# zeahmed/NeuralASR

Hardware: AMD Instinct MI355X
Metric: audio-frames/sec (fwd+bwd+CTC+Adam) at batch 16 per GPU (higher is better)
Workload: dtype f32

## Files before the change

### neuralasr_amd/csrc/lstm_persist.hip

```cpp
#include "kernels.h"
#include "lstm_device.h"

#include <cstdlib>

#ifndef NASR_PSTAMP
#define NASR_PSTAMP 0
#endif

namespace nasr {

namespace {

struct Stamps {
  unsigned long long last;
  unsigned acc[12];
  bool on;
  __device__ __forceinline__ void start(bool enable) {
    on = enable;
    for (int i = 0; i < 12; ++i) acc[i] = 0;
    last = NASR_PSTAMP ? __builtin_amdgcn_s_memtime() : 0ull;
  }
  __device__ __forceinline__ void mark(int i) {
#if NASR_PSTAMP
    if (on) {
      const unsigned long long t = __builtin_amdgcn_s_memtime();
      acc[i] += (unsigned)(t - last);
      last = t;
    }
#endif
  }
  __device__ __forceinline__ void flush(PersistCtl* ctl, unsigned slot, bool first) {
#if NASR_PSTAMP
    if (on && (threadIdx.x & 63) == 0) {
      for (int i = 0; i < 12; ++i) ctl->stamps[slot & 255][i] = acc[i];
      if (first)
        for (int i = 0; i < 12; ++i) ctl->pad[i] = acc[i];
    }
#endif
  }
};

__device__ __forceinline__ void raise_error(PersistCtl* ctl, unsigned* sticky, float* fault, unsigned code) {
  atomicOr(&ctl->error, code);
  if (fault) *fault = 1.f;
  if (sticky) __hip_atomic_store(sticky, code, __ATOMIC_RELAXED, __HIP_MEMORY_SCOPE_SYSTEM);
}

__device__ __forceinline__ bool join_group(PersistCtl* ctl, unsigned* sticky, float* fault, unsigned* info, unsigned& xcc,
                                           unsigned& member) {
  if (threadIdx.x == 0) {
    const unsigned x = __builtin_amdgcn_s_getreg((3 << 11) | 20) & 15u;
    info[0] = x;
    info[1] = x < 8 ? atomicAdd(&ctl->xcc_count[x], 1u) : 0xffffu;
    info[2] = 0;
    info[3] = 0;
    info[4] = 0;
    info[5] = 0;
  }
  __syncthreads();
  xcc = info[0];
  member = info[1];
  if (xcc >= 8 || member >= 32) {
    if (threadIdx.x == 0) raise_error(ctl, sticky, fault, 2u);
    return false;
  }
  return true;
}

}

struct RepackOffs { long long o[PERSIST_MAX_MATS]; };
__global__ __launch_bounds__(256) void repack_persist_kernel(const float* __restrict__ P, RepackOffs off,
                                                             float* __restrict__ Upf0, float* __restrict__ Upb0,
                                                             long long imf, long long imb, int Hp,
                                                             const float* __restrict__ cs0) {
  const float* __restrict__ U = P + off.o[blockIdx.y];
  float* __restrict__ Upf = Upf0 + (size_t)blockIdx.y * imf;
  float* __restrict__ Upb = Upb0 + (size_t)blockIdx.y * imb;
  const int NU = Hp / 32, KW = 8 * NU, N4 = 4 * Hp;
  const int NOG = (KW + 63) / 64, KB = NOG * 4 * NU;
  const int64_t nf = (int64_t)32 * 4 * KW * 64, nb = (int64_t)32 * 4 * KB * 64;
  const int64_t nfe = cs0 ? nf / 4 : nf;
  (void)nb; (void)Upb; (void)KB;
  for (int64_t e0 = blockIdx.x * (int64_t)blockDim.x + threadIdx.x; e0 < nfe; e0 += (int64_t)gridDim.x * blockDim.x) {
    {
      const int lane = e0 & 63;
      int64_t x = e0 >> 6;
      const int KWe = cs0 ? KW / 4 : KW;
      const int idx = (int)(x % KWe) * (cs0 ? 4 : 1); x /= KWe;
      const int w = (int)(x & 3), m = (int)(x >> 2);
      const int bp = lane >> 2, g = lane & 3;
      if (!cs0) {
        Upf[e0] = bp < NU ? U[(size_t)(w * KW + idx) * N4 + 4 * (NU * m + bp) + g] : 0.f;
      } else {
        const int col = 4 * (NU * m + bp) + g;
        const float sc = bp < NU ? cs0[(size_t)blockIdx.y * N4 + col] : 1.f;
        typedef _Float16 h4 __attribute__((ext_vector_type(4)));
        h4 p1, p2;
#pragma unroll
        for (int r = 0; r < 4; ++r) {
          const float v = bp < NU ? U[(size_t)(w * KW + idx + r) * N4 + col] * sc : 0.f;
          const _Float16 h1 = (_Float16)v;
          p1[r] = h1;
          p2[r] = (_Float16)(v - (float)h1);
        }
        h4* dst = reinterpret_cast<h4*>(Upf) + ((((size_t)m * 4 + w) * (KW / 4) + idx / 4) * 2) * 64 + lane;
        dst[0] = p1;
        dst[64] = p2;
      }
    }
  }
}

__global__ __launch_bounds__(256) void repack_persist_bwd_kernel(const float* __restrict__ P, RepackOffs off,
                                                                 float* __restrict__ Upb0, long long imb, int Hp) {
  __shared__ float tile[64][65];
  const float* __restrict__ U = P + off.o[blockIdx.y];
  float* __restrict__ Upb = Upb0 + (size_t)blockIdx.y * imb;
  const int NU = Hp / 32, KW = 8 * NU, N4 = 4 * Hp, NC = 4 * NU;
  const int NOG = (KW + 63) / 64, KB = NOG * NC;
  const int og = blockIdx.x % NOG, w = (blockIdx.x / NOG) & 3, m = blockIdx.x / (NOG * 4);
  const int cx = threadIdx.x & 63, ry = threadIdx.x >> 6;
  for (int r = ry; r < 64; r += 4) {
    const int kl = og * 64 + r;
    tile[r][cx] = (kl < KW && cx < NC) ? U[(size_t)(w * KW + kl) * N4 + NC * m + cx] : 0.f;
  }
  __syncthreads();
  float* dst = Upb + (((size_t)m * 4 + w) * KB + (size_t)og * NC) * 64;
  for (int c = ry; c < NC; c += 4) dst[(size_t)c * 64 + cx] = tile[cx][c];
}

size_t persist_image_floats(int Hp, bool bwd) {
  const int NU = Hp / 32, KW = 8 * NU, NOG = (KW + 63) / 64;
  return (size_t)32 * 4 * 64 * (bwd ? NOG * 4 * NU : KW);
}

void launch_repack_persist(const float* P, const int64_t* offs, int n, float* Upf, float* Upb, int Hp, const float* col_scale,
                           hipStream_t st) {
  const long long imf = (long long)persist_image_floats(Hp, false), imb = (long long)persist_image_floats(Hp, true);
  for (int k0 = 0; k0 < n; k0 += PERSIST_MAX_MATS) {
    const int m = n - k0 < PERSIST_MAX_MATS ? n - k0 : PERSIST_MAX_MATS;
    RepackOffs off{};
    for (int k = 0; k < m; ++k) off.o[k] = offs[k0 + k];
    hipLaunchKernelGGL(repack_persist_kernel, dim3(512, m), dim3(256), 0, st, P, off, Upf + (size_t)k0 * imf,
                       Upb + (size_t)k0 * imb, imf, imb, Hp, col_scale ? col_scale + (size_t)k0 * 4 * Hp : nullptr);
    const int NU = Hp / 32, NOG = (8 * NU + 63) / 64;
    hipLaunchKernelGGL(repack_persist_bwd_kernel, dim3(32 * 4 * NOG, m), dim3(256), 0, st, P, off, Upb + (size_t)k0 * imb, imb, Hp);
  }
}

struct PersistGeom {
  int T, Bp, Hp, D;
  int ub;
  int rounds;
  int inject;
  float* fault;
};

constexpr int PERSIST_LDS_BYTES = 96 * 1024;
constexpr int PERSIST_LDS_LEAN = 24 * 1024;

constexpr int LDS_RED = 0, LDS_ADG = 2 * 4 * 4 * 64, LDS_SIDE = LDS_ADG + 2 * 256, LDS_XGB = LDS_SIDE + 2 * 64 * 8,
              LDS_PFB = LDS_XGB + 2 * 64 * 4, LDS_INFO = LDS_PFB + 2 * 64 * 8;


template <int NU, bool F16>
__global__ __launch_bounds__(320, 1) void lstm_persist_fwd_kernel(
    const float* __restrict__ Upf,
    float* gates, float* cbuf, float* out, const int* __restrict__ seq_len,
    float* hx,
    PersistCtl* ctl, unsigned* sticky, PersistGeom gm, float fb, const float* __restrict__ cinv) {
  extern __shared__ __attribute__((aligned(16))) float lds[];
  constexpr int KW = 8 * NU;
  constexpr int NCH = 2 * NU;
  constexpr int NJ = (NCH + 15) / 16;
  constexpr bool EP = F16;
  float* red = lds + LDS_RED;
  float* side = lds + LDS_SIDE;
  float* xgb = lds + LDS_XGB;
  unsigned* info = reinterpret_cast<unsigned*>(lds + LDS_INFO);
  const int tid = threadIdx.x, w = tid >> 6, lane = tid & 63;
  unsigned xcc, member;
  if (!join_group(ctl, sticky, gm.fault, info, xcc, member)) return;
  const int T = gm.T, Bp = gm.Bp, Hp = gm.Hp, D = gm.D;
  const int NGD = 8 / D, d = (int)xcc / NGD, grp = (int)xcc % NGD;
  const int N4 = 4 * Hp, DH = D * Hp, DN = D * N4;
  if (w < 4) __builtin_amdgcn_s_setprio(3);

  typedef _Float16 h4 __attribute__((ext_vector_type(4)));
  float wreg[F16 ? 1 : KW];
  h4 w1[F16 ? KW / 4 : 1], w2[F16 ? KW / 4 : 1];
  float oscale = 1.f;
  if (w < 4) {
    if constexpr (F16) {
      const h4* wp = reinterpret_cast<const h4*>(Upf) + ((((size_t)d * 32 + member) * 4 + w) * (KW / 4) * 2) * 64 + lane;
#pragma unroll
      for (int i = 0; i < KW / 4; ++i) { w1[i] = wp[(size_t)(2 * i) * 64]; w2[i] = wp[(size_t)(2 * i + 1) * 64]; }
      const int bp = lane >> 2, g = lane & 3;
      oscale = (bp < NU ? cinv[(size_t)d * 4 * gm.Hp + 4 * (NU * (int)member + bp) + g] : 1.f) * (1.f / 16384.f);
    } else {
      const float* wp = Upf + ((((size_t)d * 32 + member) * 4 + w) * KW) * 64 + lane;
#pragma unroll
      for (int i = 0; i < KW; ++i) wreg[i] = wp[(size_t)i * 64];
    }
  }
  float* ghx = hx + (size_t)xcc * 2 * Hp * 4;
  gu32* gflag = (gu32*)(ctl->flags + xcc * 128);

  const int q = lane >> 4, u = lane & 15;
  const bool lane_ok = u < NU;
  const int j = NU * (int)member + u;
  const int jcl = j < Hp ? j : Hp - 1;
  const int hidx = (j >> 2) * 16 + q * 4 + (j & 3);
  bool aborted = false;
  Stamps stp;
  stp.start(w == 0);
  auto epoch_of = [&](int rd, int s) -> unsigned { return (unsigned)(rd * ((T + 1 - (s & 1)) >> 1) + (s >> 1) + 1) & 1u; };

  for (int rd = 0; rd < gm.rounds; ++rd) {
    const int b0 = (rd * NGD + grp) * gm.ub;
    if (b0 >= Bp) continue;
    const int b = b0 + q;
    const bool rowok = lane_ok && q < gm.ub && b < Bp;
    const int bcl = b < Bp ? b : Bp - 1;
    const int len = rowok ? seq_len[b] : 0;
    const unsigned tagbase = (unsigned)(rd * T);
    float c = 0.f;
    const unsigned xoff = (unsigned)bcl * (unsigned)DN + (unsigned)(d * N4 + 4 * jcl), xstep = (unsigned)Bp * (unsigned)DN;
    auto frame_of = [&](int s) { return (rowok && s < len) ? (d ? len - 1 - s : s) : 0; };
    auto load_xg = [&](int s) { return *reinterpret_cast<const f32x4*>(gates + (xoff + (unsigned)frame_of(s) * xstep)); };
    f32x4 xg_pf = (f32x4){0.f, 0.f, 0.f, 0.f};
    if (w == 4) xg_pf = load_xg(0);
    auto store_side = [&](int s) {
      if (rowok) {
        if (s < len) {
          const float* sp = side + ((s & 1) * 64 + lane) * 8;
          const f32x4 act = *reinterpret_cast<const f32x4*>(sp);
          const float2 ch = *reinterpret_cast<const float2*>(sp + 4);
          const unsigned r = (unsigned)((d ? (len - 1 - s) : s) * Bp + b);
          *reinterpret_cast<f32x4*>(gates + (r * (unsigned)DN + (unsigned)(d * N4 + 4 * j))) = act;
          const unsigned oc = r * (unsigned)DH + (unsigned)(d * Hp + j);
          cbuf[oc] = ch.x;
          out[oc] = ch.y;
        } else {
          out[(unsigned)(s * Bp + b) * (unsigned)DH + (unsigned)(d * Hp + j)] = 0.f;
        }
      }
    };
    for (int s = 0; s < T; ++s) {
      const int par = s & 1;
      stp.mark(0);
      bool ok = true;
      if (w < 4) {
        f32x4 acc[4];
#pragma unroll
        for (int i = 0; i < 4; ++i) acc[i] = (f32x4){0.f, 0.f, 0.f, 0.f};
        f32x4 P[NJ];
#pragma unroll
        for (int i = 0; i < NJ; ++i) P[i] = (f32x4){0.f, 0.f, 0.f, 0.f};
        if constexpr (EP) {
          if (s == 0 && rd > 0) ok = poll_ge(gflag + w * 8 + (lane & 7), lane < 8, tagbase);
          if (s == gm.inject && member == 0) ok = false;
          stp.mark(1);
          if (s > 0 && ok) {
            if (w > 0) {
              const unsigned want = tagbase + (unsigned)s;
              for (unsigned n = 0; n < (1u << 26) && (int)(*(lds_vu32*)(info + 5) - want) < 0; ++n) __builtin_amdgcn_s_sleep(1);
            }
            const float* src = ghx + (size_t)((s - 1) & 1) * Hp * 4 + ((size_t)w * KW * 4 + (size_t)lane * 4);
            const unsigned eexp = epoch_of(rd, s - 1) << 30;
            const bool has0 = NCH >= 16 || lane < 4 * NCH, has1 = NJ == 2 && lane < 4 * (NCH - 16);
            bool need = true;
            ok = false;
            for (unsigned n = 0; n < SPIN_BUDGET; ++n) {
              if (need) {
                if (has0) asm volatile("global_load_dwordx4 %0, %1, off sc1" : "=&v"(P[0]) : "v"(src) : "memory");
                if constexpr (NJ == 2)
                  if (has1) asm volatile("global_load_dwordx4 %0, %1, off offset:1024 sc1" : "=&v"(P[NJ - 1]) : "v"(src) : "memory");
              }
              if constexpr (NJ == 2) asm volatile("s_waitcnt vmcnt(0)" : "+v"(P[0]), "+v"(P[NJ - 1]) : : "memory");
              else asm volatile("s_waitcnt vmcnt(0)" : "+v"(P[0]) : : "memory");
              unsigned bad = 0;
              if (has0)
                bad |= (__float_as_uint(P[0][0]) ^ eexp) | (__float_as_uint(P[0][1]) ^ eexp) | (__float_as_uint(P[0][2]) ^ eexp) |
                       (__float_as_uint(P[0][3]) ^ eexp);
              if constexpr (NJ == 2)
                if (has1)
                  bad |= (__float_as_uint(P[NJ - 1][0]) ^ eexp) | (__float_as_uint(P[NJ - 1][1]) ^ eexp) |
                         (__float_as_uint(P[NJ - 1][2]) ^ eexp) | (__float_as_uint(P[NJ - 1][3]) ^ eexp);
              need = (bad & 0x40000000u) != 0;
              if (!__any(need)) { ok = true; break; }
#if NASR_PSTAMP
              if (stp.on) stp.acc[11] += 1;
#endif
            }
          }
        } else {
        ok = poll_ge(gflag + w * 8 + (lane & 7), lane < 8, tagbase + (unsigned)s) && !(s == gm.inject && member == 0);
        stp.mark(1);
        if (s > 0 && ok) {
          const float* src = ghx + (size_t)((s - 1) & 1) * Hp * 4 + ((size_t)w * KW * 4 + (size_t)lane * 4);
          if constexpr (NCH == 32) {
            asm volatile(
                "global_load_dwordx4 %0, %2, off sc1\n\tglobal_load_dwordx4 %1, %2, off offset:1024 sc1\n\ts_waitcnt vmcnt(0)"
                : "=&v"(P[0]), "=&v"(P[1])
                : "v"(src)
                : "memory");
          } else if constexpr (NJ == 2) {
            asm volatile("global_load_dwordx4 %0, %1, off sc1" : "=&v"(P[0]) : "v"(src) : "memory");
            if (lane < 4 * (NCH - 16)) asm volatile("global_load_dwordx4 %0, %1, off offset:1024 sc1" : "=&v"(P[1]) : "v"(src) : "memory");
            asm volatile("s_waitcnt vmcnt(0)" : "+v"(P[0]), "+v"(P[1]) : : "memory");
          } else {
            if (lane < 4 * NCH)
              asm volatile("global_load_dwordx4 %0, %1, off sc1\n\ts_waitcnt vmcnt(0)" : "=&v"(P[0]) : "v"(src) : "memory");
          }
        }
        }
        if (w == 0 && lane == 0) *(lds_vu32*)(info + 4) = tagbase + (unsigned)s + 1u;
        stp.mark(2);
        if (s > 0 && ok) {
          if constexpr (F16) {
            h4 a1[NJ], a2[NJ];
#pragma unroll
            for (int i = 0; i < NJ; ++i) {
              typedef unsigned u2 __attribute__((ext_vector_type(2)));
              const unsigned d0 = __float_as_uint(P[i][0]), d1 = __float_as_uint(P[i][1]);
              const unsigned d2 = __float_as_uint(P[i][2]), d3 = __float_as_uint(P[i][3]);
              const u2 lo = {__builtin_amdgcn_perm(d1, d0, 0x05040100u), __builtin_amdgcn_perm(d3, d2, 0x05040100u)};
              const u2 hi = {__builtin_amdgcn_perm(d1, d0, 0x07060302u), __builtin_amdgcn_perm(d3, d2, 0x07060302u)};
              a1[i] = __builtin_bit_cast(h4, lo);
              a2[i] = __builtin_bit_cast(h4, (u2){hi[0] & 0xBFFFBFFFu, hi[1] & 0xBFFFBFFFu});
            }
            static_for<0, NCH>([&](auto bbc) {
              constexpr int bb = decltype(bbc)::value;
              acc[0] = __builtin_amdgcn_mfma_f32_4x4x4f16(a2[bb / 16], w1[bb], acc[0], 4, bb % 16, 0);
              acc[1] = __builtin_amdgcn_mfma_f32_4x4x4f16(a1[bb / 16], w2[bb], acc[1], 4, bb % 16, 0);
              acc[2] = __builtin_amdgcn_mfma_f32_4x4x4f16(a1[bb / 16], w1[bb], acc[2], 4, bb % 16, 0);
            });
          } else {
            static_for<0, NCH>([&](auto bbc) {
              constexpr int bb = decltype(bbc)::value;
              static_for<0, 4>([&](auto rc) {
                constexpr int r = decltype(rc)::value;
                acc[r] = __builtin_amdgcn_mfma_f32_4x4x1f32(P[bb / 16][r], wreg[bb * 4 + r], acc[r], 4, bb % 16, 0);
              });
            });
          }
        }
        if constexpr (EP) acc[0] *= 8.f;
        f32x4 sum = (acc[0] + acc[1]) + (acc[2] + acc[3]);
        if constexpr (F16) sum *= oscale;
        float* rw = red + ((par * 4 + w) * 4) * 64 + lane;
        rw[0] = sum[0]; rw[64] = sum[1]; rw[128] = sum[2]; rw[192] = sum[3];
        if (!ok) info[2 + par] = 1;
      } else {
        *reinterpret_cast<f32x4*>(xgb + (par * 64 + lane) * 4) = xg_pf;
        const unsigned want = tagbase + (unsigned)s + 1u;
        for (unsigned n = 0; n < (1u << 26) && (int)(*(lds_vu32*)(info + 4) - want) < 0; ++n)
          __builtin_amdgcn_s_sleep(1);
        if (s + 1 < T) xg_pf = load_xg(s + 1);
        if (s > 0) store_side(s - 1);
      }
      stp.mark(3);
#if NASR_PSTAMP
      if (lane == 0) info[8 + w] = (unsigned)__builtin_amdgcn_s_memtime();
#endif
      __syncthreads();
      stp.mark(4);
#if NASR_PSTAMP
      if (stp.on) for (int i = 1; i < 5; ++i) stp.acc[6 + i] += info[8 + i] - info[8];
#endif
      const unsigned abort_word = info[2 + par];
      if (w == 0) {
        const bool valid = rowok && s < len;
        float h = 0.f;
        if (lane_ok) {
          const float* rr = red + (par * 4 * 4 + q) * 64 + 4 * u;
          const f32x4 g0 = *reinterpret_cast<const f32x4*>(rr);
          const f32x4 g1 = *reinterpret_cast<const f32x4*>(rr + 256);
          const f32x4 g2 = *reinterpret_cast<const f32x4*>(rr + 512);
          const f32x4 g3 = *reinterpret_cast<const f32x4*>(rr + 768);
          const f32x4 xg = *reinterpret_cast<const f32x4*>(xgb + (par * 64 + lane) * 4);
          const f32x4 pre = xg + ((g0 + g1) + (g2 + g3));
          f32x4 act;
          act.x = sigmoidf_(pre.x);
          act.y = tanhf_(pre.y);
          act.z = sigmoidf_(pre.z + fb);
          act.w = sigmoidf_(pre.w);
          if (valid) {
            c = c * act.z + act.x * act.y;
            h = tanhf_(c) * act.w;
          }
          if constexpr (F16) {
            const float v = h * 16384.f;
            const _Float16 h1 = (_Float16)v;
            const _Float16 h2 = (_Float16)((v - (float)h1) * 0.125f);
            const unsigned pk = (unsigned)__builtin_bit_cast(unsigned short, h1) |
                                ((unsigned)__builtin_bit_cast(unsigned short, h2) << 16) | (epoch_of(rd, s) << 30);
            ghx[(size_t)par * Hp * 4 + hidx] = __uint_as_float(pk);
          } else {
            ghx[(size_t)par * Hp * 4 + hidx] = h;
          }
          float* sp = side + (par * 64 + lane) * 8;
          *reinterpret_cast<f32x4*>(sp) = act;
          *reinterpret_cast<float2*>(sp + 4) = make_float2(c, h);
        }
        stp.mark(5);
        if constexpr (EP) {
          if (lane == 0) *(lds_vu32*)(info + 5) = tagbase + (unsigned)s + 1u;
        } else {
          asm volatile("s_waitcnt vmcnt(0)" ::: "memory");
        }
        stp.mark(6);
        if (lane == 0) *(ctl->flags + xcc * 128 + member) = tagbase + (unsigned)s + 1u;
      }
      if (abort_word) { aborted = true; break; }
    }
    if (aborted) break;
    __syncthreads();
    if (w == 4) store_side(T - 1);
  }
  stp.flush(ctl, xcc * 32 + member, xcc == 0 && member == 0);
  if (aborted && tid == 0) raise_error(ctl, sticky, gm.fault, 1u);
}

template <int NU>
__global__ __launch_bounds__(320, 1) void lstm_persist_bwd_kernel(
    const float* __restrict__ Upb, const float* __restrict__ gates, float* dgbuf, const float* __restrict__ cbuf,
    const float* __restrict__ dout, const int* __restrict__ seq_len,
    float* px,
    PersistCtl* ctl, unsigned* sticky, PersistGeom gm,
    float* __restrict__ rowpart, float* __restrict__ colpart) {
  extern __shared__ __attribute__((aligned(16))) float lds[];
  constexpr int KW = 8 * NU;
  constexpr int NOG = (KW + 63) / 64;
  constexpr int NC = 4 * NU;
  constexpr int NV = (NC + 15) / 16;
  float* adg = lds + LDS_ADG;
  float* pfb = lds + LDS_PFB;
  unsigned* info = reinterpret_cast<unsigned*>(lds + LDS_INFO);
  const int tid = threadIdx.x, w = tid >> 6, lane = tid & 63;
  unsigned xcc, member;
  if (!join_group(ctl, sticky, gm.fault, info, xcc, member)) return;
  const int T = gm.T, Bp = gm.Bp, Hp = gm.Hp, D = gm.D;
  const int NGD = 8 / D, d = (int)xcc / NGD, grp = (int)xcc % NGD;
  const int N4 = 4 * Hp, DH = D * Hp, DN = D * N4;
  if (w < 4) __builtin_amdgcn_s_setprio(3);

  float wreg[NOG * NC];
  if (w < 4) {
    const float* wp = Upb + ((((size_t)d * 32 + member) * 4 + w) * (NOG * NC)) * 64 + lane;
#pragma unroll
    for (int i = 0; i < NOG * NC; ++i) wreg[i] = wp[(size_t)i * 64];
  }
  float* gpx = px + (size_t)xcc * 2 * 32 * 32 * 64;
  gu32* gflag = (gu32*)(ctl->flags + xcc * 128);

  const int q = lane & 3, u = lane >> 2;
  const bool lane_ok = u < NU;
  const int j = NU * (int)member + u;
  const int jcl = j < Hp ? j : Hp - 1;
  bool aborted = false;
  Stamps stp;
  stp.start(w == 0);
  f32x4 cmax = (f32x4){0.f, 0.f, 0.f, 0.f};
  auto epoch_of = [&](int rd, int k) -> unsigned { return (unsigned)(rd * ((T + 1 - (k & 1)) >> 1) + (k >> 1) + 1) & 1u; };

  for (int rd = 0; rd < gm.rounds; ++rd) {
    const int b0 = (rd * NGD + grp) * gm.ub;
    if (b0 >= Bp) continue;
    const int b = b0 + q;
    const bool rowok = lane_ok && q < gm.ub && b < Bp;
    const int bcl = b < Bp ? b : Bp - 1;
    const int len = rowok ? seq_len[b] : 0;
    const unsigned tagbase = (unsigned)(rd * T);
    float dc = 0.f;
    f32x4 pa = (f32x4){0.f, 0.f, 0.f, 0.f};
    f32x4 pb = (f32x4){0.f, 0.f, 0.f, 0.f};
    auto prefetch = [&](int s) {
      const bool v = rowok && s < len;
      const int tb = v ? (d ? (len - 1 - s) : s) : 0;
      const unsigned r = (unsigned)(tb * Bp + bcl);
      const unsigned rp = (v && s > 0) ? (d ? r + (unsigned)Bp : r - (unsigned)Bp) : r;
      const unsigned cj = (unsigned)(d * Hp + jcl);
      pa = *reinterpret_cast<const f32x4*>(gates + (r * (unsigned)DN + (unsigned)(d * N4 + 4 * jcl)));
      pb.x = cbuf[r * (unsigned)DH + cj];
      pb.y = cbuf[rp * (unsigned)DH + cj];
      pb.z = dout[r * (unsigned)DH + cj];
    };
    auto hand_over = [&](int k) {
      float* dst = pfb + ((k & 1) * 64 + lane) * 8;
      *reinterpret_cast<f32x4*>(dst) = pa;
      *reinterpret_cast<f32x4*>(dst + 4) = pb;
    };
    auto store_dg = [&](int k) {
      float m = 0.f;
      unsigned row = 0;
      if (rowok) {
        const int s = T - 1 - k;
        const float* ad = adg + (k & 1) * 256 + 16 * u + q;
        const f32x4 dg = (f32x4){ad[0], ad[4], ad[8], ad[12]};
        row = (unsigned)(((s < len) ? (d ? (len - 1 - s) : s) : s) * Bp + b);
        *reinterpret_cast<f32x4*>(dgbuf + (row * (unsigned)DN + (unsigned)(d * N4 + 4 * j))) = dg;
        const f32x4 ab = (f32x4){fabsf(dg.x), fabsf(dg.y), fabsf(dg.z), fabsf(dg.w)};
        cmax = (f32x4){fmaxf(cmax.x, ab.x), fmaxf(cmax.y, ab.y), fmaxf(cmax.z, ab.z), fmaxf(cmax.w, ab.w)};
        m = fmaxf(fmaxf(ab.x, ab.y), fmaxf(ab.z, ab.w));
      }
      if (rowpart) {
        m = fmaxf(m, __builtin_bit_cast(float, __builtin_amdgcn_update_dpp(0, __builtin_bit_cast(int, m), 0x124, 0xf, 0xf, false)));
        m = fmaxf(m, __builtin_bit_cast(float, __builtin_amdgcn_update_dpp(0, __builtin_bit_cast(int, m), 0x128, 0xf, 0xf, false)));
        m = fmaxf(m, __shfl_xor(m, 16));
        m = fmaxf(m, __shfl_xor(m, 32));
        if (lane < 4 && rowok) rowpart[(size_t)(d * 32 + (int)member) * ((size_t)T * Bp) + row] = m;
      }
    };
    if (w == 4) {
      prefetch(T - 1);
      hand_over(0);
      if (T > 1) prefetch(T - 2);
    }
    __syncthreads();
    for (int k = 0; k < T; ++k) {
      const int s = T - 1 - k, par = k & 1;
      stp.mark(0);
      if (w == 0) {
        bool ok = false;
        if (k == 0 && rd > 0) {
          const unsigned want = tagbase + (unsigned)k;
          for (unsigned n = 0; n < SPIN_BUDGET && !ok; ++n) {
            const unsigned v0 = __hip_atomic_load(gflag + lane, __ATOMIC_RELAXED, __HIP_MEMORY_SCOPE_AGENT);
            const unsigned v1 = __hip_atomic_load(gflag + 64 + lane, __ATOMIC_RELAXED, __HIP_MEMORY_SCOPE_AGENT);
            ok = __all((int)(v0 - want) >= 0 && (int)(v1 - want) >= 0);
          }
        } else {
          ok = true;
        }
        if (k == gm.inject && member == 0) ok = false;
        stp.mark(1);
        const bool valid = rowok && s < len;
        const float* pf = pfb + (par * 64 + lane) * 8;
        const f32x4 a = *reinterpret_cast<const f32x4*>(pf);
        const f32x4 o = *reinterpret_cast<const f32x4*>(pf + 4);
        float dhs = o.z;
        if (k > 0 && ok) {
          const float* src = gpx + ((size_t)(((k - 1) & 1) * 32 + member) * 32) * 64 + lane;
          float pv[32];
#pragma unroll
          for (int p = 0; p < 32; ++p) pv[p] = 0.f;
#define NASR_LD8(g8)                                                                                               \
  asm volatile(                                                                                                    \
      "global_load_dword %0, %8, off sc1\n\tglobal_load_dword %1, %8, off offset:256 sc1\n\t"                       \
      "global_load_dword %2, %8, off offset:512 sc1\n\tglobal_load_dword %3, %8, off offset:768 sc1\n\t"            \
      "global_load_dword %4, %8, off offset:1024 sc1\n\tglobal_load_dword %5, %8, off offset:1280 sc1\n\t"          \
      "global_load_dword %6, %8, off offset:1536 sc1\n\tglobal_load_dword %7, %8, off offset:1792 sc1"              \
      : "=&v"(pv[g8 + 0]), "=&v"(pv[g8 + 1]), "=&v"(pv[g8 + 2]), "=&v"(pv[g8 + 3]), "=&v"(pv[g8 + 4]),             \
        "=&v"(pv[g8 + 5]), "=&v"(pv[g8 + 6]), "=&v"(pv[g8 + 7])                                                    \
      : "v"(src + (size_t)(g8) * 64)                                                                               \
      : "memory")
          const unsigned eexp = epoch_of(rd, k - 1);
          bool need = lane_ok;
          bool got = false;
          for (unsigned n = 0; n < SPIN_BUDGET; ++n) {
            if (need) { NASR_LD8(0); NASR_LD8(8); NASR_LD8(16); NASR_LD8(24); }
            asm volatile("s_waitcnt vmcnt(0)"
                         : "+v"(pv[0]), "+v"(pv[1]), "+v"(pv[2]), "+v"(pv[3]), "+v"(pv[4]), "+v"(pv[5]), "+v"(pv[6]),
                           "+v"(pv[7]), "+v"(pv[8]), "+v"(pv[9]), "+v"(pv[10]), "+v"(pv[11]), "+v"(pv[12]), "+v"(pv[13]),
                           "+v"(pv[14]), "+v"(pv[15])
                         :
                         : "memory");
            asm volatile(""
                         : "+v"(pv[16]), "+v"(pv[17]), "+v"(pv[18]), "+v"(pv[19]), "+v"(pv[20]), "+v"(pv[21]), "+v"(pv[22]),
                           "+v"(pv[23]), "+v"(pv[24]), "+v"(pv[25]), "+v"(pv[26]), "+v"(pv[27]), "+v"(pv[28]), "+v"(pv[29]),
                           "+v"(pv[30]), "+v"(pv[31])
                         :
                         : "memory");
            unsigned bad;
            if (eexp) {
              unsigned a_ = 1u;
#pragma unroll
              for (int p = 0; p < 32; ++p) a_ &= __float_as_uint(pv[p]);
              bad = ~a_;
            } else {
              unsigned o_ = 0u;
#pragma unroll
              for (int p = 0; p < 32; ++p) o_ |= __float_as_uint(pv[p]);
              bad = o_;
            }
            need = lane_ok && (bad & 1u) != 0;
            if (!__any(need)) { got = true; break; }
#if NASR_PSTAMP
            if (stp.on) stp.acc[11] += 1;
#endif
          }
#undef NASR_LD8
          if (!got) ok = false;
          if (lane_ok) {
            float s0 = 0.f, s1 = 0.f, s2 = 0.f, s3 = 0.f;
#pragma unroll
            for (int p = 0; p < 32; p += 4) { s0 += pv[p]; s1 += pv[p + 1]; s2 += pv[p + 2]; s3 += pv[p + 3]; }
            dhs += (s0 + s1) + (s2 + s3);
          }
        }
        stp.mark(2);
        f32x4 dg = (f32x4){0.f, 0.f, 0.f, 0.f};
        float dcn = 0.f;
        if (valid) {
          const float tc = tanhf_(o.x);
          const float dct = dc + dhs * a.w * (1.f - tc * tc);
          dg.x = dct * a.y * a.x * (1.f - a.x);
          dg.y = dct * a.x * (1.f - a.y * a.y);
          dg.z = dct * (s > 0 ? o.y : 0.f) * a.z * (1.f - a.z);
          dg.w = dhs * tc * a.w * (1.f - a.w);
          dcn = dct * a.z;
        }
        dc = dcn;
        if (lane_ok) {
          float* ad = adg + par * 256 + 16 * u + q;
          ad[0] = dg.x; ad[4] = dg.y; ad[8] = dg.z; ad[12] = dg.w;
        }
        if (!ok) info[2 + par] = 1;
        stp.mark(3);
      } else if (w == 4) {
        if (k + 1 < T) hand_over(k + 1);
      }
      __syncthreads();
      stp.mark(4);
      const unsigned abort_word = info[2 + par];
      if (w == 4) {
        if (k + 2 < T) prefetch(T - 3 - k);
        store_dg(k);
        if (abort_word) { aborted = true; break; }
        continue;
      }
      float av[NV];
#pragma unroll
      for (int v = 0; v < NV; ++v) av[v] = (64 * v + lane < 4 * NC) ? adg[par * 256 + 64 * v + lane] : 0.f;
      constexpr int NACC = 4;
      f32x4 acc[NOG][NACC];
#pragma unroll
      for (int og = 0; og < NOG; ++og)
#pragma unroll
        for (int a = 0; a < NACC; ++a) acc[og][a] = (f32x4){0.f, 0.f, 0.f, 0.f};
      static_for<0, NC>([&](auto cc_) {
        constexpr int c = decltype(cc_)::value;
        static_for<0, NOG>([&](auto ogc) {
          constexpr int og = decltype(ogc)::value;
          acc[og][c % NACC] = __builtin_amdgcn_mfma_f32_4x4x1f32(av[c / 16], wreg[og * NC + c], acc[og][c % NACC], 4, c % 16, 0);
        });
      });
      const unsigned eb = epoch_of(rd, k);
#pragma unroll
      for (int og = 0; og < NOG; ++og) {
        f32x4 sum = (acc[og][0] + acc[og][1]) + (acc[og][2] + acc[og][3]);
#pragma unroll
        for (int i = 0; i < 4; ++i) sum[i] = __uint_as_float((__float_as_uint(sum[i]) & ~1u) | eb);
        const int kl = og * 64 + lane;
        if (kl < KW) {
          const int kk = w * KW + kl;
          float* dst = gpx + ((size_t)((par * 32 + kk / NU) * 32) + member) * 64 + 4 * (kk % NU);
          *reinterpret_cast<f32x4*>(dst) = sum;
        }
      }
      stp.mark(5);
      stp.mark(6);
      if (lane == 0) *(ctl->flags + xcc * 128 + member * 4 + w) = tagbase + (unsigned)k + 1u;
      if (abort_word) { aborted = true; break; }
    }
    if (aborted) break;
    __syncthreads();
  }
  if (w == 4 && colpart) {
#pragma unroll
    for (int i = 0; i < 4; ++i) {
      float v = cmax[i];
      v = fmaxf(v, __builtin_bit_cast(float, __builtin_amdgcn_update_dpp(0, __builtin_bit_cast(int, v), 0xB1, 0xf, 0xf, false)));
      v = fmaxf(v, __builtin_bit_cast(float, __builtin_amdgcn_update_dpp(0, __builtin_bit_cast(int, v), 0x4E, 0xf, 0xf, false)));
      cmax[i] = v;
    }
    if (q == 0 && lane_ok) *reinterpret_cast<f32x4*>(colpart + ((size_t)grp * DN + (size_t)(d * N4 + 4 * j))) = cmax;
  }
  stp.flush(ctl, xcc * 32 + member, xcc == 0 && member == 0);
  if (aborted && tid == 0) raise_error(ctl, sticky, gm.fault, 1u);
}

bool persist_supported(int Hp) {
  const int NU = Hp / 32;
  return Hp % 64 == 0 && NU >= 2 && NU <= 16;
}

static PersistGeom make_geom(const LstmDims& dm, bool bwd) {
  PersistGeom g;
  g.T = dm.T; g.Bp = dm.Bp; g.Hp = dm.Hp; g.D = dm.D;
  const int NGD = 8 / dm.D;
  g.ub = (dm.Bp + NGD - 1) / NGD;
  if (g.ub > 4) g.ub = 4;
  g.rounds = (dm.Bp + NGD * g.ub - 1) / (NGD * g.ub);
  const char* e = test_hook("NASR_PERSIST_FAULT");
  g.inject = (e && *e) ? atoi(e) : -1;
  const char* ek = test_hook("NASR_PERSIST_FAULT_KERNEL");
  if (ek && *ek && ((ek[0] == 'b') != bwd)) g.inject = -1;
  g.fault = nullptr;
  return g;
}

size_t persist_dgmax_floats(int T, int Bp, int Hp, int D) { return (size_t)D * 32 * T * Bp + (size_t)(8 / D) * D * 4 * Hp; }

size_t persist_px_bytes() { return (size_t)8 * 2 * 32 * 32 * 64 * sizeof(float); }

size_t persist_hx_bytes(int Hp) { return (size_t)8 * 2 * Hp * 4 * sizeof(float); }

size_t persist_xch_floats(int Hp) {
  const size_t f = (size_t)8 * 2 * Hp * 4, b = (size_t)8 * 2 * 32 * 32 * 64;
  return f > b ? f : b;
}

hipError_t persist_prepare() {
  hipError_t e = hipSuccess;
#define NASR_PATTR(NUV)                                                                                             \
  if (e == hipSuccess)                                                                                              \
    e = hipFuncSetAttribute(reinterpret_cast<const void*>(&lstm_persist_fwd_kernel<NUV, false>),                    \
                            hipFuncAttributeMaxDynamicSharedMemorySize, PERSIST_LDS_BYTES);                         \
  if (e == hipSuccess)                                                                                              \
    e = hipFuncSetAttribute(reinterpret_cast<const void*>(&lstm_persist_fwd_kernel<NUV, true>),                     \
                            hipFuncAttributeMaxDynamicSharedMemorySize, PERSIST_LDS_BYTES);                         \
  if (e == hipSuccess)                                                                                              \
    e = hipFuncSetAttribute(reinterpret_cast<const void*>(&lstm_persist_bwd_kernel<NUV>),                           \
                            hipFuncAttributeMaxDynamicSharedMemorySize, PERSIST_LDS_BYTES);
  NASR_PATTR(2) NASR_PATTR(4) NASR_PATTR(6) NASR_PATTR(8) NASR_PATTR(10) NASR_PATTR(12) NASR_PATTR(14) NASR_PATTR(16)
#undef NASR_PATTR
  return e;
}

void launch_lstm_persist_fwd(const LstmDims& dm, const float* Upf, const float* cinv, float* gates, float* cbuf,
                             float* out, const int* seq_len, float* xch, PersistCtl* ctl, unsigned* sticky, float* fault,
                             float forget_bias, hipStream_t st, bool ctl_zeroed) {
  PersistGeom gm = make_geom(dm, false);
  gm.fault = fault;
  if (!ctl_zeroed) (void)hipMemsetAsync(ctl, 0, sizeof(PersistCtl), st);
  if (cinv && !ctl_zeroed) (void)hipMemsetAsync(xch, 0, persist_hx_bytes(dm.Hp), st);
  dim3 grid(256), block(320);
#define NASR_PF(NUV)                                                                                                  \
  if (cinv)                                                                                                           \
    hipLaunchKernelGGL((lstm_persist_fwd_kernel<NUV, true>), grid, block, PERSIST_LDS_BYTES, st, Upf, gates, cbuf, out,   \
                       seq_len, xch, ctl, sticky, gm, forget_bias, cinv);                                               \
  else                                                                                                                \
    hipLaunchKernelGGL((lstm_persist_fwd_kernel<NUV, false>), grid, block, PERSIST_LDS_BYTES, st, Upf, gates, cbuf, out,  \
                       seq_len, xch, ctl, sticky, gm, forget_bias, cinv)
  switch (dm.Hp / 32) {
    case 2: NASR_PF(2); break;
    case 4: NASR_PF(4); break;
    case 6: NASR_PF(6); break;
    case 8: NASR_PF(8); break;
    case 10: NASR_PF(10); break;
    case 12: NASR_PF(12); break;
    case 14: NASR_PF(14); break;
    default: NASR_PF(16); break;
  }
#undef NASR_PF
}

void launch_lstm_persist_bwd(const LstmDims& dm, const float* Upb, const float* gates, float* dgbuf, const float* cbuf,
                             const float* dout, const int* seq_len, float* xch, PersistCtl* ctl, unsigned* sticky,
                             float* fault, hipStream_t st, bool ctl_zeroed, float* rowpart, float* colpart, bool lean) {
  PersistGeom gm = make_geom(dm, true);
  gm.fault = fault;
  if (!ctl_zeroed) {
    (void)hipMemsetAsync(ctl, 0, sizeof(PersistCtl), st);
    (void)hipMemsetAsync(xch, 0, persist_px_bytes(), st);
  }
  dim3 grid(256), block(320);
  const int bwd_lds = (lean && dm.Hp == 512) ? PERSIST_LDS_LEAN : PERSIST_LDS_BYTES;
#define NASR_PB(NUV)                                                                                                   \
  hipLaunchKernelGGL((lstm_persist_bwd_kernel<NUV>), grid, block, bwd_lds, st, Upb, gates, dgbuf, cbuf, dout, \
                     seq_len, xch, ctl, sticky, gm, rowpart, colpart)
  switch (dm.Hp / 32) {
    case 2: NASR_PB(2); break;
    case 4: NASR_PB(4); break;
    case 6: NASR_PB(6); break;
    case 8: NASR_PB(8); break;
    case 10: NASR_PB(10); break;
    case 12: NASR_PB(12); break;
    case 14: NASR_PB(14); break;
    default: NASR_PB(16); break;
  }
#undef NASR_PB
}

}
```

Measured before the change: 1.232 million.

## Defer LSTM cell update past barrier and stagger backward MFMA hand-off

```diff
diff --git a/neuralasr_amd/csrc/lstm_persist.hip b/neuralasr_amd/csrc/lstm_persist.hip
--- a/neuralasr_amd/csrc/lstm_persist.hip
+++ b/neuralasr_amd/csrc/lstm_persist.hip
@@ -247,8 +247,60 @@
         }
       }
     };
+    auto cell_update = [&](int s) {
+      const int par = s & 1;
+      const bool valid = rowok && s < len;
+      float h = 0.f;
+      if (lane_ok) {
+        const float* rr = red + (par * 4 * 4 + q) * 64 + 4 * u;
+        const f32x4 g0 = *reinterpret_cast<const f32x4*>(rr);
+        const f32x4 g1 = *reinterpret_cast<const f32x4*>(rr + 256);
+        const f32x4 g2 = *reinterpret_cast<const f32x4*>(rr + 512);
+        const f32x4 g3 = *reinterpret_cast<const f32x4*>(rr + 768);
+        const f32x4 xg = *reinterpret_cast<const f32x4*>(xgb + (par * 64 + lane) * 4);
+        const f32x4 pre = xg + ((g0 + g1) + (g2 + g3));
+        f32x4 act;
+        act.x = sigmoidf_(pre.x);
+        act.y = tanhf_(pre.y);
+        act.z = sigmoidf_(pre.z + fb);
+        act.w = sigmoidf_(pre.w);
+        if (valid) {
+          c = c * act.z + act.x * act.y;
+          h = tanhf_(c) * act.w;
+        }
+        if constexpr (F16) {
+          const float v = h * 16384.f;
+          const _Float16 h1 = (_Float16)v;
+          const _Float16 h2 = (_Float16)((v - (float)h1) * 0.125f);
+          const unsigned pk = (unsigned)__builtin_bit_cast(unsigned short, h1) |
+                              ((unsigned)__builtin_bit_cast(unsigned short, h2) << 16) | (epoch_of(rd, s) << 30);
+          ghx[(size_t)par * Hp * 4 + hidx] = __uint_as_float(pk);
+        } else {
+          ghx[(size_t)par * Hp * 4 + hidx] = h;
+        }
+        float* sp = side + (par * 64 + lane) * 8;
+        *reinterpret_cast<f32x4*>(sp) = act;
+        *reinterpret_cast<float2*>(sp + 4) = make_float2(c, h);
+      }
+    };
+    auto publish = [&](int s) {
+      if constexpr (EP) {
+        if (lane == 0) *(lds_vu32*)(info + 5) = tagbase + (unsigned)s + 1u;
+      } else {
+        asm volatile("s_waitcnt vmcnt(0)" ::: "memory");
+        if (lane == 0) *(ctl->flags + xcc * 128 + member) = tagbase + (unsigned)s + 1u;
+      }
+    };
+    unsigned abort_word = 0;
     for (int s = 0; s < T; ++s) {
       const int par = s & 1;
+      if (w == 0 && s > 0) {
+        cell_update(s - 1);
+        stp.mark(5);
+        publish(s - 1);
+        stp.mark(6);
+      }
+      if (abort_word) { aborted = true; break; }
       stp.mark(0);
       bool ok = true;
       if (w < 4) {
@@ -260,7 +312,7 @@
         for (int i = 0; i < NJ; ++i) P[i] = (f32x4){0.f, 0.f, 0.f, 0.f};
         if constexpr (EP) {
           if (s == 0 && rd > 0) ok = poll_ge(gflag + w * 8 + (lane & 7), lane < 8, tagbase);
-          if (s == gm.inject && member == 0) ok = false;
+          if ((int)tagbase + s == gm.inject && member == 0) ok = false;
           stp.mark(1);
           if (s > 0 && ok) {
             if (w > 0) {
@@ -296,7 +348,7 @@
             }
           }
         } else {
-        ok = poll_ge(gflag + w * 8 + (lane & 7), lane < 8, tagbase + (unsigned)s) && !(s == gm.inject && member == 0);
+        ok = poll_ge(gflag + w * 8 + (lane & 7), lane < 8, tagbase + (unsigned)s) && !((int)tagbase + s == gm.inject && member == 0);
         stp.mark(1);
         if (s > 0 && ok) {
           const float* src = ghx + (size_t)((s - 1) & 1) * Hp * 4 + ((size_t)w * KW * 4 + (size_t)lane * 4);
@@ -370,53 +422,15 @@
 #if NASR_PSTAMP
       if (stp.on) for (int i = 1; i < 5; ++i) stp.acc[6 + i] += info[8 + i] - info[8];
 #endif
-      const unsigned abort_word = info[2 + par];
-      if (w == 0) {
-        const bool valid = rowok && s < len;
-        float h = 0.f;
-        if (lane_ok) {
-          const float* rr = red + (par * 4 * 4 + q) * 64 + 4 * u;
-          const f32x4 g0 = *reinterpret_cast<const f32x4*>(rr);
-          const f32x4 g1 = *reinterpret_cast<const f32x4*>(rr + 256);
-          const f32x4 g2 = *reinterpret_cast<const f32x4*>(rr + 512);
-          const f32x4 g3 = *reinterpret_cast<const f32x4*>(rr + 768);
-          const f32x4 xg = *reinterpret_cast<const f32x4*>(xgb + (par * 64 + lane) * 4);
-          const f32x4 pre = xg + ((g0 + g1) + (g2 + g3));
-          f32x4 act;
-          act.x = sigmoidf_(pre.x);
-          act.y = tanhf_(pre.y);
-          act.z = sigmoidf_(pre.z + fb);
-          act.w = sigmoidf_(pre.w);
-          if (valid) {
-            c = c * act.z + act.x * act.y;
-            h = tanhf_(c) * act.w;
-          }
-          if constexpr (F16) {
-            const float v = h * 16384.f;
-            const _Float16 h1 = (_Float16)v;
-            const _Float16 h2 = (_Float16)((v - (float)h1) * 0.125f);
-            const unsigned pk = (unsigned)__builtin_bit_cast(unsigned short, h1) |
-                                ((unsigned)__builtin_bit_cast(unsigned short, h2) << 16) | (epoch_of(rd, s) << 30);
-            ghx[(size_t)par * Hp * 4 + hidx] = __uint_as_float(pk);
-          } else {
-            ghx[(size_t)par * Hp * 4 + hidx] = h;
-          }
-          float* sp = side + (par * 64 + lane) * 8;
-          *reinterpret_cast<f32x4*>(sp) = act;
-          *reinterpret_cast<float2*>(sp + 4) = make_float2(c, h);
-        }
-        stp.mark(5);
-        if constexpr (EP) {
-          if (lane == 0) *(lds_vu32*)(info + 5) = tagbase + (unsigned)s + 1u;
-        } else {
-          asm volatile("s_waitcnt vmcnt(0)" ::: "memory");
-        }
-        stp.mark(6);
-        if (lane == 0) *(ctl->flags + xcc * 128 + member) = tagbase + (unsigned)s + 1u;
-      }
-      if (abort_word) { aborted = true; break; }
+      abort_word = info[2 + par];
     }
     if (aborted) break;
+    if (w == 0) {
+      cell_update(T - 1);
+      if constexpr (!EP) asm volatile("s_waitcnt vmcnt(0)" ::: "memory");
+      if (lane == 0) *(ctl->flags + xcc * 128 + member) = tagbase + (unsigned)T;
+    }
+    if (abort_word) { aborted = true; break; }
     __syncthreads();
     if (w == 4) store_side(T - 1);
   }
@@ -535,7 +549,7 @@
         } else {
           ok = true;
         }
-        if (k == gm.inject && member == 0) ok = false;
+        if ((int)tagbase + k == gm.inject && member == 0) ok = false;
         stp.mark(1);
         const bool valid = rowok && s < len;
         const float* pf = pfb + (par * 64 + lane) * 8;
@@ -641,16 +655,8 @@
       for (int og = 0; og < NOG; ++og)
 #pragma unroll
         for (int a = 0; a < NACC; ++a) acc[og][a] = (f32x4){0.f, 0.f, 0.f, 0.f};
-      static_for<0, NC>([&](auto cc_) {
-        constexpr int c = decltype(cc_)::value;
-        static_for<0, NOG>([&](auto ogc) {
-          constexpr int og = decltype(ogc)::value;
-          acc[og][c % NACC] = __builtin_amdgcn_mfma_f32_4x4x1f32(av[c / 16], wreg[og * NC + c], acc[og][c % NACC], 4, c % 16, 0);
-        });
-      });
       const unsigned eb = epoch_of(rd, k);
-#pragma unroll
-      for (int og = 0; og < NOG; ++og) {
+      auto hand_off = [&](int og) {
         f32x4 sum = (acc[og][0] + acc[og][1]) + (acc[og][2] + acc[og][3]);
 #pragma unroll
         for (int i = 0; i < 4; ++i) sum[i] = __uint_as_float((__float_as_uint(sum[i]) & ~1u) | eb);
@@ -660,10 +666,38 @@
           float* dst = gpx + ((size_t)((par * 32 + kk / NU) * 32) + member) * 64 + 4 * (kk % NU);
           *reinterpret_cast<f32x4*>(dst) = sum;
         }
+      };
+      if constexpr (NOG == 2) {
+        constexpr int LAG = 16;
+        static_assert(NC > LAG, "both groups overlap for NC - LAG products");
+        static_for<0, NC + LAG>([&](auto ic) {
+          constexpr int i = decltype(ic)::value;
+          if constexpr (i < NC)
+            acc[0][i % NACC] = __builtin_amdgcn_mfma_f32_4x4x1f32(av[i / 16], wreg[i], acc[0][i % NACC], 4, i % 16, 0);
+          if constexpr (i >= LAG) {
+            constexpr int c = i - LAG;
+            acc[1][c % NACC] = __builtin_amdgcn_mfma_f32_4x4x1f32(av[c / 16], wreg[NC + c], acc[1][c % NACC], 4, c % 16, 0);
+          }
+          if constexpr (i == NC - 1 + 4) {
+            __builtin_amdgcn_sched_barrier(0);
+            hand_off(0);
+          }
+        });
+        hand_off(1);
+      } else {
+        static_for<0, NC>([&](auto cc_) {
+          constexpr int c = decltype(cc_)::value;
+          static_for<0, NOG>([&](auto ogc) {
+            constexpr int og = decltype(ogc)::value;
+            acc[og][c % NACC] = __builtin_amdgcn_mfma_f32_4x4x1f32(av[c / 16], wreg[og * NC + c], acc[og][c % NACC], 4, c % 16, 0);
+          });
+        });
+#pragma unroll
+        for (int og = 0; og < NOG; ++og) hand_off(og);
       }
       stp.mark(5);
       stp.mark(6);
-      if (lane == 0) *(ctl->flags + xcc * 128 + member * 4 + w) = tagbase + (unsigned)k + 1u;
+      if (lane == 0 && k == T - 1) *(ctl->flags + xcc * 128 + member * 4 + w) = tagbase + (unsigned)T;
       if (abort_word) { aborted = true; break; }
     }
     if (aborted) break;
```

New measurement: 1.247 million, median of 6. 1.01x the previous value.
